# kwea123/nerf_pl

Hardware: AMD Instinct MI355X
Metric: rays/sec (64+128 samples), full training step: render_rays fwd + MSE + bwd + grad all-reduce + Adam (higher is better)
Workload: dtype bf16

## Files before the change

### nerf_pl_amd/csrc/composite_wave.h

```cpp
#pragma once
#include "loss_math.h"
#include "sampling_wave.h"

namespace nerfhip {

struct RayGeom {
    float dnorm;
};

__device__ __forceinline__ float ray_dnorm(const float* __restrict__ rays, int64_t r) {
    const float dx = rays[r * 8 + 3], dy = rays[r * 8 + 4], dz = rays[r * 8 + 5];
    return sqrtf(nh_add(nh_add(nh_mul(dx, dx), nh_mul(dy, dy)), nh_mul(dz, dz)));
}

struct SampleTerms {
    float delta;
    float e;
    float alpha;
    float sh;
    bool on;
};

__device__ __forceinline__ SampleTerms sample_terms(float z_i, float z_next, bool last, float dnorm, float sigma,
                                                    float noise) {
    SampleTerms t;
    const float d = last ? 1e10f : nh_sub(z_next, z_i);
    t.delta = nh_mul(d, dnorm);
    const float s = nh_add(sigma, noise);
    t.on = s > 0.0f;
    const float sr = t.on ? s : 0.0f;
    t.e = expf(-nh_mul(t.delta, sr));
    t.alpha = nh_sub(1.0f, t.e);
    t.sh = nh_add(nh_sub(1.0f, t.alpha), 1e-10f);
    return t;
}

template <int RAW_CH>
__device__ __forceinline__ void composite_fwd_wave(const float* __restrict__ raw, const float* __restrict__ z,
                                                   const float* __restrict__ rays, const float* __restrict__ noise, float noise_std,
                                                   int white_back, float* __restrict__ weights, float* __restrict__ rgb,
                                                   float* __restrict__ depth, float* __restrict__ opacity, int64_t r, int S,
                                                   float* w_s, int lane) {
    const float dnorm = ray_dnorm(rays, r);
    const float* zr = z + r * S;
    double carry = 1.0;
    float acc_r = 0.f, acc_g = 0.f, acc_b = 0.f, acc_d = 0.f, acc_o = 0.f;
    for (int i0 = 0; i0 < S; i0 += 64) {
        const int i = i0 + lane;
        const bool valid = i < S;
        float sigma = 0.f, cr = 0.f, cg = 0.f, cb = 0.f, zi = 0.f, zn = 0.f, nz = 0.f;
        if (valid) {
            zi = zr[i];
            zn = (i + 1 < S) ? zr[i + 1] : zi;
            if (RAW_CH == 4) {
                const float4 v = reinterpret_cast<const float4*>(raw)[r * S + i];
                cr = v.x; cg = v.y; cb = v.z; sigma = v.w;
            } else {
                sigma = raw[r * S + i];
            }
            if (noise) nz = nh_mul(noise[r * S + i], noise_std);
        }
        const SampleTerms t = sample_terms(zi, zn, i == S - 1, dnorm, sigma, nz);
        const double f = valid ? (double)t.sh : 1.0;
        const double incl = wave_incl_prod(f, lane);
        double excl = __shfl_up(incl, 1, 64);
        if (lane == 0) excl = 1.0;
        const float T = (float)(excl * carry);
        carry = carry * __shfl(incl, 63, 64);
        const float w = valid ? nh_mul(t.alpha, T) : 0.0f;
        if (valid) {
            if (weights) weights[r * S + i] = w;
            if (w_s) w_s[i] = w;
        }
        acc_o += w;
        if (RAW_CH == 4) {
            acc_r += w * cr; acc_g += w * cg; acc_b += w * cb;
            acc_d += w * zi;
        }
    }
    acc_o = wave_sum(acc_o);
    if (RAW_CH == 4) {
        acc_r = wave_sum(acc_r); acc_g = wave_sum(acc_g); acc_b = wave_sum(acc_b); acc_d = wave_sum(acc_d);
    }
    if (lane == 0) {
        if (opacity) opacity[r] = acc_o;
        if (RAW_CH == 4) {
            const float bg = white_back ? nh_sub(1.0f, acc_o) : 0.0f;
            if (rgb) {
                rgb[r * 3 + 0] = acc_r + bg;
                rgb[r * 3 + 1] = acc_g + bg;
                rgb[r * 3 + 2] = acc_b + bg;
            }
            if (depth) depth[r] = acc_d;
        }
    }
}

template <bool RGB_THROUGH = false>
__device__ __forceinline__ void composite_train_wave(const float* __restrict__ raw, const float* __restrict__ z,
                                                     const float* __restrict__ rays, const float* __restrict__ noise,
                                                     float noise_std, int white_back, const float* __restrict__ target,
                                                     float gscale, float* __restrict__ weights, float* __restrict__ rgb,
                                                     float* __restrict__ depth, float* __restrict__ opacity,
                                                     float* __restrict__ g_raw, int64_t r, int S, float* T_s, float* w_s, int lane) {
    const float dnorm = ray_dnorm(rays, r);
    const float* zr = z + r * S;
    double carry = 1.0;
    float acc_r = 0.f, acc_g = 0.f, acc_b = 0.f, acc_d = 0.f, acc_o = 0.f;
    for (int i0 = 0; i0 < S; i0 += 64) {
        const int i = i0 + lane;
        const bool valid = i < S;
        float sigma = 0.f, cr = 0.f, cg = 0.f, cb = 0.f, zi = 0.f, zn = 0.f, nz = 0.f;
        if (valid) {
            zi = zr[i];
            zn = (i + 1 < S) ? zr[i + 1] : zi;
            const float4 v = reinterpret_cast<const float4*>(raw)[r * S + i];
            cr = v.x; cg = v.y; cb = v.z; sigma = v.w;
            if (noise) nz = nh_mul(noise[r * S + i], noise_std);
        }
        const SampleTerms t = sample_terms(zi, zn, i == S - 1, dnorm, sigma, nz);
        const double f = valid ? (double)t.sh : 1.0;
        const double incl = wave_incl_prod(f, lane);
        double excl = __shfl_up(incl, 1, 64);
        if (lane == 0) excl = 1.0;
        const float T = (float)(excl * carry);
        carry = carry * __shfl(incl, 63, 64);
        const float w = valid ? nh_mul(t.alpha, T) : 0.0f;
        if (valid) {
            if (weights) weights[r * S + i] = w;
            if (w_s) w_s[i] = w;
            T_s[i] = T;
        }
        acc_o += w;
        acc_r += w * cr; acc_g += w * cg; acc_b += w * cb;
        acc_d += w * zi;
    }
    acc_o = wave_sum(acc_o);
    acc_r = wave_sum(acc_r); acc_g = wave_sum(acc_g); acc_b = wave_sum(acc_b); acc_d = wave_sum(acc_d);
    const float bg = white_back ? nh_sub(1.0f, acc_o) : 0.0f;
    const float out_r = acc_r + bg, out_g = acc_g + bg, out_b = acc_b + bg;
    if (lane == 0) {
        opacity[r] = acc_o;
        if (RGB_THROUGH) {
            __hip_atomic_store(rgb + r * 3 + 0, out_r, __ATOMIC_RELAXED, __HIP_MEMORY_SCOPE_AGENT);
            __hip_atomic_store(rgb + r * 3 + 1, out_g, __ATOMIC_RELAXED, __HIP_MEMORY_SCOPE_AGENT);
            __hip_atomic_store(rgb + r * 3 + 2, out_b, __ATOMIC_RELAXED, __HIP_MEMORY_SCOPE_AGENT);
        } else {
            rgb[r * 3 + 0] = out_r;
            rgb[r * 3 + 1] = out_g;
            rgb[r * 3 + 2] = out_b;
        }
        depth[r] = acc_d;
    }
    const float gr = nh_mul(nh_sub(out_r, target[r * 3]), gscale);
    const float gg = nh_mul(nh_sub(out_g, target[r * 3 + 1]), gscale);
    const float gb = nh_mul(nh_sub(out_b, target[r * 3 + 2]), gscale);
    const float gd = 0.f;
    float gconst = 0.f;
    if (white_back) gconst -= (gr + gg + gb);
    __builtin_amdgcn_wave_barrier();
    float tail = 0.f;
    const int nchunk = (S + 63) / 64;
    for (int c = nchunk - 1; c >= 0; --c) {
        const int i = c * 64 + lane;
        const bool valid = i < S;
        SampleTerms t{};
        float T = 0.f, gw = 0.f;
        if (valid) {
            const float zi = zr[i];
            const float zn = (i + 1 < S) ? zr[i + 1] : zi;
            const float4 v = reinterpret_cast<const float4*>(raw)[r * S + i];
            const float nz = noise ? nh_mul(noise[r * S + i], noise_std) : 0.f;
            t = sample_terms(zi, zn, i == S - 1, dnorm, v.w, nz);
            T = T_s[i];
            const float w = t.alpha * T;
            gw = gconst + 0.f;
            gw += gr * v.x + gg * v.y + gb * v.z + gd * zi;
            float* o = g_raw + (r * S + i) * 4;
            o[0] = w * gr; o[1] = w * gg; o[2] = w * gb;
        }
        const float vv = valid ? gw * (t.alpha * T) : 0.f;
        float incl = vv;
#pragma unroll
        for (int o = 1; o < 64; o <<= 1) {
            const float tt = __shfl_down(incl, o, 64);
            if (lane + o < 64) incl += tt;
        }
        const float suf = (incl - vv) + tail;
        tail += __shfl(incl, 0, 64);
        if (valid) {
            const float g_alpha = gw * T - suf / t.sh;
            const float g_sigma = t.on ? g_alpha * t.delta * t.e : 0.f;
            g_raw[(r * S + i) * 4 + 3] = g_sigma;
        }
    }
}

template <int RAW_CH = 4>
__device__ __forceinline__ void composite_weights_wave(const float* __restrict__ raw, const float* __restrict__ z,
                                                       const float* __restrict__ rays, const float* __restrict__ noise,
                                                       float noise_std, int64_t r, int S, float* w_s, int lane) {
    const float dnorm = ray_dnorm(rays, r);
    const float* zr = z + r * S;
    double carry = 1.0;
    for (int i0 = 0; i0 < S; i0 += 64) {
        const int i = i0 + lane;
        const bool valid = i < S;
        float sigma = 0.f, zi = 0.f, zn = 0.f, nz = 0.f;
        if (valid) {
            zi = zr[i];
            zn = (i + 1 < S) ? zr[i + 1] : zi;
            sigma = RAW_CH == 4 ? raw[(r * S + i) * 4 + 3] : raw[r * S + i];
            if (noise) nz = nh_mul(noise[r * S + i], noise_std);
        }
        const SampleTerms t = sample_terms(zi, zn, i == S - 1, dnorm, sigma, nz);
        const double f = valid ? (double)t.sh : 1.0;
        const double incl = wave_incl_prod(f, lane);
        double excl = __shfl_up(incl, 1, 64);
        if (lane == 0) excl = 1.0;
        const float T = (float)(excl * carry);
        carry = carry * __shfl(incl, 63, 64);
        if (valid) w_s[i] = nh_mul(t.alpha, T);
    }
}

}
```

### nerf_pl_amd/csrc/mlp_render_kernel.h

```cpp
#pragma once
#include "composite_wave.h"
#include "mlp_fwd_kernel.h"

namespace nerfhip {

constexpr int kRenderRays = 4;

typedef nerfhip_render_args RenderArgs;

__host__ __device__ inline int render_tail_floats(int S_c, int N_i, int S_f) {
    const int S4 = (S_c + 3) & ~3, N4 = (N_i + 3) & ~3, F4 = (S_f + 3) & ~3;
    const int fz = N_i > 0 ? 3 * S4 + N4 + ((S_c + 1 + 3) & ~3) + N4 : 0;
    const int coarse = 2 * S4 + fz;
    return coarse > F4 ? coarse : F4;
}

__device__ __forceinline__ void render_wg_sync() {
    asm volatile("s_waitcnt vmcnt(0) lgkmcnt(0)\n\ts_barrier" ::: "memory");
}

typedef const RenderArgs __attribute__((address_space(4)))* RenderArgsP;
__device__ __forceinline__ RenderArgsP render_args() {
    RenderArgsP p = (RenderArgsP)__builtin_amdgcn_kernarg_segment_ptr();
    asm volatile("" : "+s"(p));
    return p;
}

template <bool TRAIN, int NW, bool TT = false>
__device__ __forceinline__ void render_tail(const bool fine_pass, const bool with_fine_z, float* const tail_lds, const int wave,
                                            const int lane) {
    constexpr int R = kRenderRays;
    const RenderArgsP a = render_args();
    const int S_c = a->S_c, N_i = a->N_i, S_f = S_c + N_i;
    const float noise_std = a->noise_std;
    const float* raw = fine_pass ? a->raw_fine : a->raw_coarse;
    const float* z = fine_pass ? a->z_fine : a->z_coarse;
    const float* noise = noise_std != 0.0f ? (fine_pass ? a->noise_fine : a->noise_coarse) : nullptr;
    const int S = fine_pass ? S_f : S_c;
    float* rgb = fine_pass ? a->rgb_fine : a->rgb_coarse;
    float* depth = fine_pass ? a->depth_fine : a->depth_coarse;
    float* opac = fine_pass ? a->opacity_fine : a->opacity_coarse;
    const float* rays = a->rays;
    const int white_back = a->white_back;
    const int per_ray = render_tail_floats(S_c, N_i, S_f);
    const int S4 = (S_c + 3) & ~3;
    const int64_t ray0 = (int64_t)blockIdx.x * R, B = a->B;
    const int njobs = with_fine_z ? 2 * R : R;
    for (int job = wave; job < njobs; job += NW) {
        const int slot = job < R ? job : job - R;
        const int64_t r = ray0 + slot;
        if (r >= B) continue;
        float* base = tail_lds + (size_t)slot * per_ray;
        if (job < R) {
            if constexpr (TRAIN) {
                composite_train_wave<true>(raw, z, rays, noise, noise_std, white_back, a->target, a->grad_scale, nullptr, rgb, depth, opac,
                                           fine_pass ? a->g_raw_fine : a->g_raw_coarse, r, S, base, nullptr, lane);
            } else if (TT && !fine_pass) {
                composite_fwd_wave<1>(raw, z, rays, noise, noise_std, white_back, nullptr, nullptr, nullptr, opac, r, S, nullptr, lane);
            } else {
                composite_fwd_wave<4>(raw, z, rays, noise, noise_std, white_back, nullptr, rgb, depth, opac, r, S, nullptr, lane);
            }
        } else {
            float* w_s = base + S4;
            composite_weights_wave<(TT ? 1 : 4)>(raw, z, rays, noise, noise_std, r, S, w_s, lane);
            __builtin_amdgcn_wave_barrier();
            const float* u = a->u;
            fine_z_wave(w_s + S4, z + r * S, [&](int j) { return w_s[1 + j]; }, u ? u + r * a->u_stride : nullptr, S, N_i, a->eps,
                        a->z_fine + r * S_f, nullptr, nullptr, nullptr, lane, a->row_total);
        }
    }
}

template <int PREC, int SV>
__global__ __launch_bounds__(PrecTraits<PREC>::NW * 64, PrecTraits<PREC>::WPS)
void mlp_render_kernel(const RenderArgs args_by_value) {
    constexpr bool TRAIN = SV == 1 || SV == 2, TT = SV == 3;
    constexpr int FSV = TT ? 0 : SV;
    constexpr int NW = PrecTraits<PREC>::NW, PTS = 32 * NW, R = kRenderRays;
    __shared__ __attribute__((aligned(1024))) char lds_all[FwdLds<PREC, TRAIN>::kBytes];
    __shared__ float red[2][16];
    __shared__ unsigned last_s;
    const int lane = threadIdx.x & 63;
    const int wave = __builtin_amdgcn_readfirstlane((int)(threadIdx.x >> 6));
    float* const tail_lds = reinterpret_cast<float*>(lds_all + FwdLds<PREC, TRAIN>::kRingOff);
    int nc, nf;
    {
        const RenderArgsP a = render_args();
        const int S_c = a->S_c, N_i = a->N_i;
        nc = R * S_c / PTS;
        nf = N_i > 0 ? R * (S_c + N_i) / PTS : 0;
    }
    const int total = nc + nf;
#pragma clang loop unroll(disable)
    for (int sp = 0; sp < total; ++sp) {
        if (sp > 0) render_wg_sync();
        if (sp == nc) {
            render_tail<TRAIN, NW, TT>(false, true, tail_lds, wave, lane);
            render_wg_sync();
        }
        const RenderArgsP a = render_args();
        const bool fine = sp >= nc;
        const int S = fine ? a->S_c + a->N_i : a->S_c;
        const unsigned blk = fine ? blockIdx.x * (unsigned)nf + (unsigned)(sp - nc) : blockIdx.x * (unsigned)nc + (unsigned)sp;
        const FwdZGen zg{fine ? nullptr : a->perturb_rand, fine ? nullptr : a->z_coarse, fine ? 0 : a->use_disp, fine ? 0.0f : a->perturb,
                          TRAIN ? a->regen_enc : 0};
        uint8_t* save = nullptr;
        if constexpr (TRAIN) save = (uint8_t*)(fine ? a->save_fine : a->save_coarse);
        if (TT && !fine)
            mlp_fwd_body<PREC, MODE_RAYS, true, 0>(lds_all, blk, a->rays, nullptr, a->B * (int64_t)S, (int64_t)S, (const uint8_t*)a->packed_coarse,
                                                   a->raw_coarse, nullptr, zg);
        else
            mlp_fwd_body<PREC, MODE_RAYS, false, FSV>(lds_all, blk, a->rays, fine ? a->z_fine : nullptr, a->B * (int64_t)S, (int64_t)S,
                                                      (const uint8_t*)(fine ? a->packed_fine : a->packed_coarse), fine ? a->raw_fine : a->raw_coarse, save, zg);
    }
    render_wg_sync();
    render_tail<TRAIN, NW, TT>(nf > 0, false, tail_lds, wave, lane);

    if constexpr (TRAIN) {
        const RenderArgsP a = render_args();
        unsigned* const ticket = a->ticket;
        asm volatile("s_waitcnt vmcnt(0)" ::: "memory");
        __syncthreads();
        if (threadIdx.x == 0) {
            const unsigned prev = __hip_atomic_fetch_add(ticket, 1u, __ATOMIC_RELAXED, __HIP_MEMORY_SCOPE_AGENT);
            last_s = (prev == gridDim.x - 1) ? 1u : 0u;
            if (prev == gridDim.x - 1) __hip_atomic_store(ticket, 0u, __ATOMIC_RELAXED, __HIP_MEMORY_SCOPE_AGENT);
        }
        __syncthreads();
        if (!last_s) return;
        __builtin_amdgcn_fence(__ATOMIC_ACQUIRE, "agent");
        const float* img_c = a->rgb_coarse;
        const float* img_f = a->rgb_fine;
        const float* target = a->target;
        float* out3 = a->out3;
        const int64_t n3 = 3 * a->B;
        auto fresh_c = [&](int64_t i) { return __hip_atomic_load(img_c + i, __ATOMIC_RELAXED, __HIP_MEMORY_SCOPE_AGENT); };
        auto fresh_f = [&](int64_t i) { return __hip_atomic_load(img_f + i, __ATOMIC_RELAXED, __HIP_MEMORY_SCOPE_AGENT); };
        constexpr int Q = 1024 / (NW * 64);
        if (nf > 0)
            mse_psnr_block<Q>(fresh_c, fresh_f, true, target, n3, out3, nullptr, nullptr, red);
        else
            mse_psnr_block<Q>(fresh_c, [&](int64_t i) { return 0.0f; }, false, target, n3, out3, nullptr, nullptr, red);
    }
}

template <int PREC, int SV>
int launch_render_variant(const RenderArgs& a, unsigned groups, hipStream_t stream);

}
```

### nerf_pl_amd/csrc/optim.hip

```cpp
#include "adam_math.h"

namespace nerfhip {

constexpr int kAdamMaxTensors = 8;
struct AdamTable {
    float* param[kAdamMaxTensors];
    const float* grad[kAdamMaxTensors];
    float* m[kAdamMaxTensors];
    float* v[kAdamMaxTensors];
    int64_t n[kAdamMaxTensors];
    int block0[kAdamMaxTensors + 1];
    int count;
};

constexpr int kAdamThreads = 256, kAdamVec = 4, kAdamPerBlock = kAdamThreads * kAdamVec * 4;

__device__ __forceinline__ void advance_step(float* state, float t) {
    __syncthreads();
    if (threadIdx.x == 0) {
        unsigned* ticket = reinterpret_cast<unsigned*>(state + 1);
        const unsigned prev = atomicAdd(ticket, 1u);
        if (prev == gridDim.x - 1) {
            *ticket = 0u;
            state[0] = t;
        }
    }
}

__global__ __launch_bounds__(kAdamThreads) void adam_kernel(AdamTable T, float* __restrict__ state, float lr, float beta1,
                                                            float beta2, float eps, float wd) {
    const float t = state[0] + 1.0f;
    int ti = 0;
#pragma unroll
    for (int k = 1; k < kAdamMaxTensors; ++k) ti += (k < T.count && (int)blockIdx.x >= T.block0[k]) ? 1 : 0;
    const int64_t base = (int64_t)((int)blockIdx.x - T.block0[ti]) * kAdamPerBlock;
    const int64_t n = T.n[ti];
    float* __restrict__ P = T.param[ti];
    const float* __restrict__ G = T.grad[ti];
    float* __restrict__ M = T.m[ti];
    float* __restrict__ V = T.v[ti];
    const AdamCoef ac = adam_coef(t, lr, beta1, beta2);
#pragma unroll
    for (int r = 0; r < 4; ++r) {
        const int64_t i = base + ((int64_t)r * kAdamThreads + threadIdx.x) * kAdamVec;
        if (i + kAdamVec <= n && ((((uintptr_t)(P + i)) | ((uintptr_t)(G + i)) | ((uintptr_t)(M + i)) | ((uintptr_t)(V + i))) & 15) == 0) {
            float4 p = *reinterpret_cast<const float4*>(P + i), g = *reinterpret_cast<const float4*>(G + i);
            float4 m = *reinterpret_cast<const float4*>(M + i), v = *reinterpret_cast<const float4*>(V + i);
            float* pp = &p.x; float* gp = &g.x; float* mp = &m.x; float* vp = &v.x;
#pragma unroll
            for (int k = 0; k < 4; ++k) adam_elem(pp[k], gp[k], mp[k], vp[k], ac, beta2, eps, wd);
            *reinterpret_cast<float4*>(P + i) = p;
            *reinterpret_cast<float4*>(M + i) = m;
            *reinterpret_cast<float4*>(V + i) = v;
        } else {
            for (int k = 0; k < kAdamVec; ++k) {
                const int64_t j = i + k;
                if (j < n) adam_elem(P[j], G[j], M[j], V[j], ac, beta2, eps, wd);
            }
        }
    }
    __syncthreads();
    if (threadIdx.x == 0) {
        unsigned* ticket = reinterpret_cast<unsigned*>(state + 1);
        const unsigned prev = atomicAdd(ticket, 1u);
        if (prev == gridDim.x - 1) {
            *ticket = 0u;
            state[0] = t;
        }
    }
}

struct SlowTable {
    float* slow[kAdamMaxTensors];
};

struct RadamCoef {
    float step_lr;
    float wd_lr;
    float beta1, beta2, omb1, omb2, eps, alpha;
    int mode;
    bool decay, sync, init;
};

template <bool kRanger>
__device__ __forceinline__ RadamCoef radam_coef(float t, double lr, double beta1, double beta2, double eps, double wd, double alpha,
                                                int k, double threshold, int degenerated_to_sgd) {
    RadamCoef c;
    const double td = (double)t;
    const double beta2_t = pow(beta2, td);
    const double n_max = 2.0 / (1.0 - beta2) - 1.0;
    const double n_sma = n_max - 2.0 * td * beta2_t / (1.0 - beta2_t);
    const double bc1 = 1.0 - pow(beta1, td);
    const bool rectified = kRanger ? (n_sma > threshold) : (n_sma >= threshold);
    double step_size;
    if (rectified) {
        step_size = sqrt((1.0 - beta2_t) * (n_sma - 4.0) / (n_max - 4.0) * (n_sma - 2.0) / n_sma * n_max / (n_max - 2.0)) / bc1;
        c.mode = 2;
    } else {
        step_size = 1.0 / bc1;
        c.mode = (kRanger || degenerated_to_sgd) ? 1 : 0;
    }
    c.step_lr = (float)(-step_size * lr);
    c.wd_lr = (float)(-wd * lr);
    c.decay = wd != 0.0;
    c.beta1 = (float)beta1;
    c.beta2 = (float)beta2;
    c.omb1 = (float)(1.0 - beta1);
    c.omb2 = (float)(1.0 - beta2);
    c.eps = (float)eps;
    c.alpha = (float)alpha;
    c.sync = kRanger && ((int)t % k == 0);
    c.init = kRanger && t == 1.0f;
    return c;
}

template <bool kRanger>
__device__ __forceinline__ void radam_elem(float& p, float g, float& m, float& v, float& s, const RadamCoef& c) {
    v = v * c.beta2 + c.omb2 * g * g;
    m = m * c.beta1 + c.omb1 * g;
    if (c.mode == 0) return;
    float q = p;
    if (kRanger && c.init) s = q;
    if (c.decay) q = q + c.wd_lr * q;
    q = (c.mode == 2) ? q + c.step_lr * (m / (sqrtf(v) + c.eps)) : q + c.step_lr * m;
    if (kRanger && c.sync) {
        s = s + c.alpha * (q - s);
        q = s;
    }
    p = q;
}

template <bool kRanger>
__global__ __launch_bounds__(kAdamThreads) void radam_kernel(AdamTable T, SlowTable ST, float* __restrict__ state, double lr,
                                                             double beta1, double beta2, double eps, double wd, double alpha, int k,
                                                             double threshold, int degenerated_to_sgd) {
    const float t = state[0] + 1.0f;
    int ti = 0;
#pragma unroll
    for (int j = 1; j < kAdamMaxTensors; ++j) ti += (j < T.count && (int)blockIdx.x >= T.block0[j]) ? 1 : 0;
    const int64_t base = (int64_t)((int)blockIdx.x - T.block0[ti]) * kAdamPerBlock;
    const int64_t n = T.n[ti];
    float* __restrict__ P = T.param[ti];
    const float* __restrict__ G = T.grad[ti];
    float* __restrict__ M = T.m[ti];
    float* __restrict__ V = T.v[ti];
    const RadamCoef c = radam_coef<kRanger>(t, lr, beta1, beta2, eps, wd, alpha, k, threshold, degenerated_to_sgd);
    const bool slow_rd = kRanger && c.sync && !c.init, slow_wr = kRanger && (c.sync || c.init);
    float* __restrict__ S = slow_wr ? ST.slow[ti] : nullptr;
#pragma unroll
    for (int r = 0; r < 4; ++r) {
        const int64_t i = base + ((int64_t)r * kAdamThreads + threadIdx.x) * kAdamVec;
        uintptr_t align = ((uintptr_t)(P + i)) | ((uintptr_t)(G + i)) | ((uintptr_t)(M + i)) | ((uintptr_t)(V + i));
        if (slow_wr) align |= (uintptr_t)(S + i);
        if (i + kAdamVec <= n && (align & 15) == 0) {
            float4 p = *reinterpret_cast<const float4*>(P + i), g = *reinterpret_cast<const float4*>(G + i);
            float4 m = *reinterpret_cast<const float4*>(M + i), v = *reinterpret_cast<const float4*>(V + i);
            float4 s = make_float4(0.f, 0.f, 0.f, 0.f);
            if (slow_rd) s = *reinterpret_cast<const float4*>(S + i);
            float* pp = &p.x; float* gp = &g.x; float* mp = &m.x; float* vp = &v.x; float* sp = &s.x;
#pragma unroll
            for (int e = 0; e < 4; ++e) radam_elem<kRanger>(pp[e], gp[e], mp[e], vp[e], sp[e], c);
            if (c.mode != 0) *reinterpret_cast<float4*>(P + i) = p;
            *reinterpret_cast<float4*>(M + i) = m;
            *reinterpret_cast<float4*>(V + i) = v;
            if (slow_wr) *reinterpret_cast<float4*>(S + i) = s;
        } else {
            for (int e = 0; e < kAdamVec; ++e) {
                const int64_t j = i + e;
                if (j < n) {
                    float p = P[j], m = M[j], v = V[j], s = slow_rd ? S[j] : 0.f;
                    radam_elem<kRanger>(p, G[j], m, v, s, c);
                    if (c.mode != 0) P[j] = p;
                    M[j] = m;
                    V[j] = v;
                    if (slow_wr) S[j] = s;
                }
            }
        }
    }
    advance_step(state, t);
}

}

namespace nerfhip {

static int adam_table(AdamTable& T, int& blocks, float* const* params_host, const float* const* grads_host, float* const* exp_avg_host,
                      float* const* exp_avg_sq_host, const int64_t* numel_host, int n_tensors) {
    NERFHIP_CHECK_ARG(params_host && grads_host && exp_avg_host && exp_avg_sq_host && numel_host);
    NERFHIP_CHECK_ARG(n_tensors >= 1 && n_tensors <= kAdamMaxTensors);
    blocks = 0;
    for (int i = 0; i < n_tensors; ++i) {
        NERFHIP_CHECK_ARG(params_host[i] && grads_host[i] && exp_avg_host[i] && exp_avg_sq_host[i] && numel_host[i] > 0);
        T.param[i] = params_host[i];
        T.grad[i] = grads_host[i];
        T.m[i] = exp_avg_host[i];
        T.v[i] = exp_avg_sq_host[i];
        T.n[i] = numel_host[i];
        T.block0[i] = blocks;
        const int64_t nb = (numel_host[i] + kAdamPerBlock - 1) / kAdamPerBlock;
        if (nb + blocks > 0x3fffffff) return NERFHIP_E_BADARG;
        blocks += (int)nb;
    }
    for (int i = n_tensors; i < kAdamMaxTensors; ++i) {
        T.param[i] = nullptr; T.grad[i] = nullptr; T.m[i] = nullptr; T.v[i] = nullptr; T.n[i] = 0;
        T.block0[i] = blocks;
    }
    T.block0[kAdamMaxTensors] = blocks;
    T.count = n_tensors;
    return 0;
}

static bool radam_hyper_ok(double lr, double beta1, double beta2, double eps, double weight_decay) {
    return lr >= 0.0 && beta1 >= 0.0 && beta1 < 1.0 && beta2 >= 0.0 && beta2 < 1.0 && eps >= 0.0 && weight_decay >= 0.0;
}

}

extern "C" int nerfhip_adam_step(float* const* params_host, const float* const* grads_host, float* const* exp_avg_host,
                                 float* const* exp_avg_sq_host, const int64_t* numel_host, int n_tensors, float* state,
                                 float lr, float beta1, float beta2, float eps, float weight_decay, nerfhip_stream_t stream) {
    NERFHIP_CHECK_ARG(state);
    nerfhip::AdamTable T;
    int blocks = 0;
    const int rc = nerfhip::adam_table(T, blocks, params_host, grads_host, exp_avg_host, exp_avg_sq_host, numel_host, n_tensors);
    if (rc != 0) return rc;
    hipLaunchKernelGGL(nerfhip::adam_kernel, dim3(blocks), dim3(nerfhip::kAdamThreads), 0, (hipStream_t)stream, T, state, lr,
                       beta1, beta2, eps, weight_decay);
    return nerfhip_launch_status();
}

extern "C" int nerfhip_radam_step(float* const* params_host, const float* const* grads_host, float* const* exp_avg_host,
                                  float* const* exp_avg_sq_host, const int64_t* numel_host, int n_tensors, float* state,
                                  double lr, double beta1, double beta2, double eps, double weight_decay, int degenerated_to_sgd,
                                  nerfhip_stream_t stream) {
    NERFHIP_CHECK_ARG(state && nerfhip::radam_hyper_ok(lr, beta1, beta2, eps, weight_decay));
    nerfhip::AdamTable T;
    int blocks = 0;
    const int rc = nerfhip::adam_table(T, blocks, params_host, grads_host, exp_avg_host, exp_avg_sq_host, numel_host, n_tensors);
    if (rc != 0) return rc;
    nerfhip::SlowTable ST;
    for (int i = 0; i < nerfhip::kAdamMaxTensors; ++i) ST.slow[i] = nullptr;
    hipLaunchKernelGGL(nerfhip::radam_kernel<false>, dim3(blocks), dim3(nerfhip::kAdamThreads), 0, (hipStream_t)stream, T, ST, state,
                       lr, beta1, beta2, eps, weight_decay, 0.0, 1, 5.0, degenerated_to_sgd ? 1 : 0);
    return nerfhip_launch_status();
}

extern "C" int nerfhip_ranger_step(float* const* params_host, const float* const* grads_host, float* const* exp_avg_host,
                                   float* const* exp_avg_sq_host, const int64_t* numel_host, int n_tensors, float* state,
                                   float* const* slow_host, double alpha, int k, double n_sma_threshold, double lr, double beta1,
                                   double beta2, double eps, double weight_decay, nerfhip_stream_t stream) {
    NERFHIP_CHECK_ARG(state && slow_host && nerfhip::radam_hyper_ok(lr, beta1, beta2, eps, weight_decay));
    NERFHIP_CHECK_ARG(k >= 1 && alpha >= 0.0 && alpha <= 1.0);
    nerfhip::AdamTable T;
    int blocks = 0;
    const int rc = nerfhip::adam_table(T, blocks, params_host, grads_host, exp_avg_host, exp_avg_sq_host, numel_host, n_tensors);
    if (rc != 0) return rc;
    nerfhip::SlowTable ST;
    for (int i = 0; i < nerfhip::kAdamMaxTensors; ++i) {
        ST.slow[i] = i < n_tensors ? slow_host[i] : nullptr;
        NERFHIP_CHECK_ARG(i >= n_tensors || slow_host[i]);
    }
    hipLaunchKernelGGL(nerfhip::radam_kernel<true>, dim3(blocks), dim3(nerfhip::kAdamThreads), 0, (hipStream_t)stream, T, ST, state,
                       lr, beta1, beta2, eps, weight_decay, alpha, k, n_sma_threshold, 1);
    return nerfhip_launch_status();
}
```

Baseline: 1.096 million.

## Batch composite loads across sample chunks and hoist Adam loads ahead of math

The composite forward, train and weights routines now load several 64-sample chunks of z, raw and noise into registers up front (clamped indices, masked afterwards), instead of issuing guarded loads one chunk at a time. When all samples fit in one group, the backward pass reuses the registers filled by the forward pass rather than reloading from global memory. The Adam kernel gets a whole-block fast path that issues all 16 float4 loads before any math and pins them with empty asm to keep loads early, aiming to expose more memory-level parallelism. An optional timestamp probe is also added behind a compile flag that is off by default. The cost is higher register pressure, which may lower occupancy.

```diff
diff --git a/nerf_pl_amd/csrc/composite_wave.h b/nerf_pl_amd/csrc/composite_wave.h
--- a/nerf_pl_amd/csrc/composite_wave.h
+++ b/nerf_pl_amd/csrc/composite_wave.h
@@ -35,8 +35,42 @@
     return t;
 }
 
-template <int RAW_CH>
-__device__ __forceinline__ void composite_fwd_wave(const float* __restrict__ raw, const float* __restrict__ z,
+constexpr int kCompositeGroup = 4;
+template <int RAW_CH, int NC>
+struct CompositeChunks {
+    float4 v[NC];
+    float zi[NC], zn[NC], nz[NC];
+    template <bool SIGMA_ONLY, bool NOISE>
+    __device__ __forceinline__ void load_all(const float* __restrict__ raw, const float* __restrict__ zr, const float* __restrict__ noise,
+                                             float noise_std, int64_t r, int S, int g0, int lane) {
+#pragma unroll
+        for (int c = 0; c < NC; ++c) {
+            const int i = g0 + 64 * c + lane;
+            const int ic = i < S ? i : S - 1, in = i + 1 < S ? i + 1 : S - 1;
+            zi[c] = zr[ic];
+            zn[c] = zr[in];
+            if (RAW_CH == 4 && !SIGMA_ONLY) v[c] = reinterpret_cast<const float4*>(raw)[r * S + ic];
+            else v[c] = make_float4(0.f, 0.f, 0.f, RAW_CH == 4 ? raw[(r * S + ic) * 4 + 3] : raw[r * S + ic]);
+            nz[c] = NOISE ? noise[r * S + ic] : 0.f;
+        }
+#pragma unroll
+        for (int c = 0; c < NC; ++c) {
+            const bool valid = g0 + 64 * c + lane < S;
+            if (NOISE) nz[c] = nh_mul(nz[c], noise_std);
+            zi[c] = valid ? zi[c] : 0.f; zn[c] = valid ? zn[c] : 0.f; nz[c] = valid ? nz[c] : 0.f;
+            v[c].x = valid ? v[c].x : 0.f; v[c].y = valid ? v[c].y : 0.f; v[c].z = valid ? v[c].z : 0.f; v[c].w = valid ? v[c].w : 0.f;
+        }
+    }
+    template <bool SIGMA_ONLY = false>
+    __device__ __forceinline__ void load(const float* __restrict__ raw, const float* __restrict__ zr, const float* __restrict__ noise,
+                                         float noise_std, int64_t r, int S, int g0, int lane) {
+        if (noise) load_all<SIGMA_ONLY, true>(raw, zr, noise, noise_std, r, S, g0, lane);
+        else load_all<SIGMA_ONLY, false>(raw, zr, noise, noise_std, r, S, g0, lane);
+    }
+};
+
+template <int RAW_CH, int NC>
+__device__ __forceinline__ void composite_fwd_wave_impl(const float* __restrict__ raw, const float* __restrict__ z,
                                                    const float* __restrict__ rays, const float* __restrict__ noise, float noise_std,
                                                    int white_back, float* __restrict__ weights, float* __restrict__ rgb,
                                                    float* __restrict__ depth, float* __restrict__ opacity, int64_t r, int S,
@@ -45,37 +79,33 @@
     const float* zr = z + r * S;
     double carry = 1.0;
     float acc_r = 0.f, acc_g = 0.f, acc_b = 0.f, acc_d = 0.f, acc_o = 0.f;
-    for (int i0 = 0; i0 < S; i0 += 64) {
-        const int i = i0 + lane;
-        const bool valid = i < S;
-        float sigma = 0.f, cr = 0.f, cg = 0.f, cb = 0.f, zi = 0.f, zn = 0.f, nz = 0.f;
-        if (valid) {
-            zi = zr[i];
-            zn = (i + 1 < S) ? zr[i + 1] : zi;
+    CompositeChunks<RAW_CH, NC> in;
+    for (int g0 = 0; g0 < S; g0 += 64 * NC) {
+        in.load(raw, zr, noise, noise_std, r, S, g0, lane);
+#pragma unroll
+        for (int c = 0; c < NC; ++c) {
+            const int i0 = g0 + 64 * c;
+            if (i0 >= S) break;
+            const int i = i0 + lane;
+            const bool valid = i < S;
+            const float cr = in.v[c].x, cg = in.v[c].y, cb = in.v[c].z, sigma = in.v[c].w, zi = in.zi[c];
+            const SampleTerms t = sample_terms(zi, in.zn[c], i == S - 1, dnorm, sigma, in.nz[c]);
+            const double f = valid ? (double)t.sh : 1.0;
+            const double incl = wave_incl_prod(f, lane);
+            double excl = __shfl_up(incl, 1, 64);
+            if (lane == 0) excl = 1.0;
+            const float T = (float)(excl * carry);
+            carry = carry * __shfl(incl, 63, 64);
+            const float w = valid ? nh_mul(t.alpha, T) : 0.0f;
+            if (valid) {
+                if (weights) weights[r * S + i] = w;
+                if (w_s) w_s[i] = w;
+            }
+            acc_o += w;
             if (RAW_CH == 4) {
-                const float4 v = reinterpret_cast<const float4*>(raw)[r * S + i];
-                cr = v.x; cg = v.y; cb = v.z; sigma = v.w;
-            } else {
-                sigma = raw[r * S + i];
-            }
-            if (noise) nz = nh_mul(noise[r * S + i], noise_std);
-        }
-        const SampleTerms t = sample_terms(zi, zn, i == S - 1, dnorm, sigma, nz);
-        const double f = valid ? (double)t.sh : 1.0;
-        const double incl = wave_incl_prod(f, lane);
-        double excl = __shfl_up(incl, 1, 64);
-        if (lane == 0) excl = 1.0;
-        const float T = (float)(excl * carry);
-        carry = carry * __shfl(incl, 63, 64);
-        const float w = valid ? nh_mul(t.alpha, T) : 0.0f;
-        if (valid) {
-            if (weights) weights[r * S + i] = w;
-            if (w_s) w_s[i] = w;
-        }
-        acc_o += w;
-        if (RAW_CH == 4) {
-            acc_r += w * cr; acc_g += w * cg; acc_b += w * cb;
-            acc_d += w * zi;
+                acc_r += w * cr; acc_g += w * cg; acc_b += w * cb;
+                acc_d += w * zi;
+            }
         }
     }
     acc_o = wave_sum(acc_o);
@@ -95,9 +125,18 @@
         }
     }
 }
-
-template <bool RGB_THROUGH = false>
-__device__ __forceinline__ void composite_train_wave(const float* __restrict__ raw, const float* __restrict__ z,
+template <int RAW_CH>
+__device__ __forceinline__ void composite_fwd_wave(const float* __restrict__ raw, const float* __restrict__ z,
+                                                   const float* __restrict__ rays, const float* __restrict__ noise, float noise_std,
+                                                   int white_back, float* __restrict__ weights, float* __restrict__ rgb,
+                                                   float* __restrict__ depth, float* __restrict__ opacity, int64_t r, int S,
+                                                   float* w_s, int lane) {
+    if (S <= 64) composite_fwd_wave_impl<RAW_CH, 1>(raw, z, rays, noise, noise_std, white_back, weights, rgb, depth, opacity, r, S, w_s, lane);
+    else composite_fwd_wave_impl<RAW_CH, kCompositeGroup>(raw, z, rays, noise, noise_std, white_back, weights, rgb, depth, opacity, r, S, w_s, lane);
+}
+
+template <bool RGB_THROUGH, int NC>
+__device__ __forceinline__ void composite_train_wave_impl(const float* __restrict__ raw, const float* __restrict__ z,
                                                      const float* __restrict__ rays, const float* __restrict__ noise,
                                                      float noise_std, int white_back, const float* __restrict__ target,
                                                      float gscale, float* __restrict__ weights, float* __restrict__ rgb,
@@ -105,35 +144,37 @@
                                                      float* __restrict__ g_raw, int64_t r, int S, float* T_s, float* w_s, int lane) {
     const float dnorm = ray_dnorm(rays, r);
     const float* zr = z + r * S;
+    const float tgt_r = target[r * 3], tgt_g = target[r * 3 + 1], tgt_b = target[r * 3 + 2];
     double carry = 1.0;
     float acc_r = 0.f, acc_g = 0.f, acc_b = 0.f, acc_d = 0.f, acc_o = 0.f;
-    for (int i0 = 0; i0 < S; i0 += 64) {
-        const int i = i0 + lane;
-        const bool valid = i < S;
-        float sigma = 0.f, cr = 0.f, cg = 0.f, cb = 0.f, zi = 0.f, zn = 0.f, nz = 0.f;
-        if (valid) {
-            zi = zr[i];
-            zn = (i + 1 < S) ? zr[i + 1] : zi;
-            const float4 v = reinterpret_cast<const float4*>(raw)[r * S + i];
-            cr = v.x; cg = v.y; cb = v.z; sigma = v.w;
-            if (noise) nz = nh_mul(noise[r * S + i], noise_std);
-        }
-        const SampleTerms t = sample_terms(zi, zn, i == S - 1, dnorm, sigma, nz);
-        const double f = valid ? (double)t.sh : 1.0;
-        const double incl = wave_incl_prod(f, lane);
-        double excl = __shfl_up(incl, 1, 64);
-        if (lane == 0) excl = 1.0;
-        const float T = (float)(excl * carry);
-        carry = carry * __shfl(incl, 63, 64);
-        const float w = valid ? nh_mul(t.alpha, T) : 0.0f;
-        if (valid) {
-            if (weights) weights[r * S + i] = w;
-            if (w_s) w_s[i] = w;
-            T_s[i] = T;
-        }
-        acc_o += w;
-        acc_r += w * cr; acc_g += w * cg; acc_b += w * cb;
-        acc_d += w * zi;
+    CompositeChunks<4, NC> in;
+    const bool one_group = S <= 64 * NC;
+    for (int g0 = 0; g0 < S; g0 += 64 * NC) {
+        in.load(raw, zr, noise, noise_std, r, S, g0, lane);
+#pragma unroll
+        for (int c = 0; c < NC; ++c) {
+            const int i0 = g0 + 64 * c;
+            if (i0 >= S) break;
+            const int i = i0 + lane;
+            const bool valid = i < S;
+            const float cr = in.v[c].x, cg = in.v[c].y, cb = in.v[c].z, sigma = in.v[c].w, zi = in.zi[c];
+            const SampleTerms t = sample_terms(zi, in.zn[c], i == S - 1, dnorm, sigma, in.nz[c]);
+            const double f = valid ? (double)t.sh : 1.0;
+            const double incl = wave_incl_prod(f, lane);
+            double excl = __shfl_up(incl, 1, 64);
+            if (lane == 0) excl = 1.0;
+            const float T = (float)(excl * carry);
+            carry = carry * __shfl(incl, 63, 64);
+            const float w = valid ? nh_mul(t.alpha, T) : 0.0f;
+            if (valid) {
+                if (weights) weights[r * S + i] = w;
+                if (w_s) w_s[i] = w;
+                T_s[i] = T;
+            }
+            acc_o += w;
+            acc_r += w * cr; acc_g += w * cg; acc_b += w * cb;
+            acc_d += w * zi;
+        }
     }
     acc_o = wave_sum(acc_o);
     acc_r = wave_sum(acc_r); acc_g = wave_sum(acc_g); acc_b = wave_sum(acc_b); acc_d = wave_sum(acc_d);
@@ -152,76 +193,102 @@
         }
         depth[r] = acc_d;
     }
-    const float gr = nh_mul(nh_sub(out_r, target[r * 3]), gscale);
-    const float gg = nh_mul(nh_sub(out_g, target[r * 3 + 1]), gscale);
-    const float gb = nh_mul(nh_sub(out_b, target[r * 3 + 2]), gscale);
+    const float gr = nh_mul(nh_sub(out_r, tgt_r), gscale);
+    const float gg = nh_mul(nh_sub(out_g, tgt_g), gscale);
+    const float gb = nh_mul(nh_sub(out_b, tgt_b), gscale);
     const float gd = 0.f;
     float gconst = 0.f;
     if (white_back) gconst -= (gr + gg + gb);
     __builtin_amdgcn_wave_barrier();
     float tail = 0.f;
-    const int nchunk = (S + 63) / 64;
-    for (int c = nchunk - 1; c >= 0; --c) {
-        const int i = c * 64 + lane;
-        const bool valid = i < S;
-        SampleTerms t{};
-        float T = 0.f, gw = 0.f;
-        if (valid) {
-            const float zi = zr[i];
-            const float zn = (i + 1 < S) ? zr[i + 1] : zi;
-            const float4 v = reinterpret_cast<const float4*>(raw)[r * S + i];
-            const float nz = noise ? nh_mul(noise[r * S + i], noise_std) : 0.f;
-            t = sample_terms(zi, zn, i == S - 1, dnorm, v.w, nz);
-            T = T_s[i];
-            const float w = t.alpha * T;
-            gw = gconst + 0.f;
-            gw += gr * v.x + gg * v.y + gb * v.z + gd * zi;
-            float* o = g_raw + (r * S + i) * 4;
-            o[0] = w * gr; o[1] = w * gg; o[2] = w * gb;
-        }
-        const float vv = valid ? gw * (t.alpha * T) : 0.f;
-        float incl = vv;
-#pragma unroll
-        for (int o = 1; o < 64; o <<= 1) {
-            const float tt = __shfl_down(incl, o, 64);
-            if (lane + o < 64) incl += tt;
-        }
-        const float suf = (incl - vv) + tail;
-        tail += __shfl(incl, 0, 64);
-        if (valid) {
-            const float g_alpha = gw * T - suf / t.sh;
-            const float g_sigma = t.on ? g_alpha * t.delta * t.e : 0.f;
-            g_raw[(r * S + i) * 4 + 3] = g_sigma;
-        }
-    }
-}
-
-template <int RAW_CH = 4>
-__device__ __forceinline__ void composite_weights_wave(const float* __restrict__ raw, const float* __restrict__ z,
+    const int ngroup = (S + 64 * NC - 1) / (64 * NC);
+    for (int g = ngroup - 1; g >= 0; --g) {
+        const int g0 = g * 64 * NC;
+        if (!one_group) in.load(raw, zr, noise, noise_std, r, S, g0, lane);
+#pragma unroll
+        for (int c = NC - 1; c >= 0; --c) {
+            const int i0 = g0 + 64 * c;
+            if (i0 >= S) continue;
+            const int i = i0 + lane;
+            const bool valid = i < S;
+            SampleTerms t{};
+            float T = 0.f, gw = 0.f;
+            if (valid) {
+                const float zi = in.zi[c];
+                const float4 v = in.v[c];
+                t = sample_terms(zi, in.zn[c], i == S - 1, dnorm, v.w, in.nz[c]);
+                T = T_s[i];
+                const float w = t.alpha * T;
+                gw = gconst + 0.f;
+                gw += gr * v.x + gg * v.y + gb * v.z + gd * zi;
+                float* o = g_raw + (r * S + i) * 4;
+                o[0] = w * gr; o[1] = w * gg; o[2] = w * gb;
+            }
+            const float vv = valid ? gw * (t.alpha * T) : 0.f;
+            float incl = vv;
+#pragma unroll
+            for (int o = 1; o < 64; o <<= 1) {
+                const float tt = __shfl_down(incl, o, 64);
+                if (lane + o < 64) incl += tt;
+            }
+            const float suf = (incl - vv) + tail;
+            tail += __shfl(incl, 0, 64);
+            if (valid) {
+                const float g_alpha = gw * T - suf / t.sh;
+                const float g_sigma = t.on ? g_alpha * t.delta * t.e : 0.f;
+                g_raw[(r * S + i) * 4 + 3] = g_sigma;
+            }
+        }
+    }
+}
+template <bool RGB_THROUGH = false>
+__device__ __forceinline__ void composite_train_wave(const float* __restrict__ raw, const float* __restrict__ z,
+                                                     const float* __restrict__ rays, const float* __restrict__ noise,
+                                                     float noise_std, int white_back, const float* __restrict__ target,
+                                                     float gscale, float* __restrict__ weights, float* __restrict__ rgb,
+                                                     float* __restrict__ depth, float* __restrict__ opacity,
+                                                     float* __restrict__ g_raw, int64_t r, int S, float* T_s, float* w_s, int lane) {
+    if (S <= 64)
+        composite_train_wave_impl<RGB_THROUGH, 1>(raw, z, rays, noise, noise_std, white_back, target, gscale, weights, rgb, depth, opacity, g_raw,
+                                                  r, S, T_s, w_s, lane);
+    else
+        composite_train_wave_impl<RGB_THROUGH, kCompositeGroup>(raw, z, rays, noise, noise_std, white_back, target, gscale, weights, rgb, depth,
+                                                                opacity, g_raw, r, S, T_s, w_s, lane);
+}
+
+template <int RAW_CH, int NC>
+__device__ __forceinline__ void composite_weights_wave_impl(const float* __restrict__ raw, const float* __restrict__ z,
                                                        const float* __restrict__ rays, const float* __restrict__ noise,
                                                        float noise_std, int64_t r, int S, float* w_s, int lane) {
     const float dnorm = ray_dnorm(rays, r);
     const float* zr = z + r * S;
     double carry = 1.0;
-    for (int i0 = 0; i0 < S; i0 += 64) {
-        const int i = i0 + lane;
-        const bool valid = i < S;
-        float sigma = 0.f, zi = 0.f, zn = 0.f, nz = 0.f;
-        if (valid) {
-            zi = zr[i];
-            zn = (i + 1 < S) ? zr[i + 1] : zi;
-            sigma = RAW_CH == 4 ? raw[(r * S + i) * 4 + 3] : raw[r * S + i];
-            if (noise) nz = nh_mul(noise[r * S + i], noise_std);
-        }
-        const SampleTerms t = sample_terms(zi, zn, i == S - 1, dnorm, sigma, nz);
-        const double f = valid ? (double)t.sh : 1.0;
-        const double incl = wave_incl_prod(f, lane);
-        double excl = __shfl_up(incl, 1, 64);
-        if (lane == 0) excl = 1.0;
-        const float T = (float)(excl * carry);
-        carry = carry * __shfl(incl, 63, 64);
-        if (valid) w_s[i] = nh_mul(t.alpha, T);
-    }
-}
-
-}
+    CompositeChunks<RAW_CH, NC> in;
+    for (int g0 = 0; g0 < S; g0 += 64 * NC) {
+        in.template load<true>(raw, zr, noise, noise_std, r, S, g0, lane);
+#pragma unroll
+        for (int c = 0; c < NC; ++c) {
+            const int i0 = g0 + 64 * c;
+            if (i0 >= S) break;
+            const int i = i0 + lane;
+            const bool valid = i < S;
+            const SampleTerms t = sample_terms(in.zi[c], in.zn[c], i == S - 1, dnorm, in.v[c].w, in.nz[c]);
+            const double f = valid ? (double)t.sh : 1.0;
+            const double incl = wave_incl_prod(f, lane);
+            double excl = __shfl_up(incl, 1, 64);
+            if (lane == 0) excl = 1.0;
+            const float T = (float)(excl * carry);
+            carry = carry * __shfl(incl, 63, 64);
+            if (valid) w_s[i] = nh_mul(t.alpha, T);
+        }
+    }
+}
+template <int RAW_CH = 4>
+__device__ __forceinline__ void composite_weights_wave(const float* __restrict__ raw, const float* __restrict__ z,
+                                                       const float* __restrict__ rays, const float* __restrict__ noise,
+                                                       float noise_std, int64_t r, int S, float* w_s, int lane) {
+    if (S <= 64) composite_weights_wave_impl<RAW_CH, 1>(raw, z, rays, noise, noise_std, r, S, w_s, lane);
+    else composite_weights_wave_impl<RAW_CH, kCompositeGroup>(raw, z, rays, noise, noise_std, r, S, w_s, lane);
+}
+
+}
diff --git a/nerf_pl_amd/csrc/mlp_render_kernel.h b/nerf_pl_amd/csrc/mlp_render_kernel.h
--- a/nerf_pl_amd/csrc/mlp_render_kernel.h
+++ b/nerf_pl_amd/csrc/mlp_render_kernel.h
@@ -5,6 +5,16 @@
 namespace nerfhip {
 
 constexpr int kRenderRays = 4;
+
+#ifndef NERFHIP_SEAM_PROBE
+#define NERFHIP_SEAM_PROBE 0
+#endif
+#if NERFHIP_SEAM_PROBE
+constexpr int kSeamStamps = 24;
+#define NERFHIP_SEAM_STAMP(k) do { if (lane == 0) seam_s[wave][(k)] = (unsigned)__builtin_amdgcn_s_memrealtime(); } while (0)
+#else
+#define NERFHIP_SEAM_STAMP(k) do { } while (0)
+#endif
 
 typedef nerfhip_render_args RenderArgs;
 
@@ -82,6 +92,11 @@
     __shared__ unsigned last_s;
     const int lane = threadIdx.x & 63;
     const int wave = __builtin_amdgcn_readfirstlane((int)(threadIdx.x >> 6));
+#if NERFHIP_SEAM_PROBE
+    __shared__ unsigned seam_s[NW][kSeamStamps];
+    if (lane < kSeamStamps) seam_s[wave][lane] = 0u;
+    NERFHIP_SEAM_STAMP(0);
+#endif
     float* const tail_lds = reinterpret_cast<float*>(lds_all + FwdLds<PREC, TRAIN>::kRingOff);
     int nc, nf;
     {
@@ -95,8 +110,11 @@
     for (int sp = 0; sp < total; ++sp) {
         if (sp > 0) render_wg_sync();
         if (sp == nc) {
+            NERFHIP_SEAM_STAMP(9);
             render_tail<TRAIN, NW, TT>(false, true, tail_lds, wave, lane);
+            NERFHIP_SEAM_STAMP(10);
             render_wg_sync();
+            NERFHIP_SEAM_STAMP(11);
         }
         const RenderArgsP a = render_args();
         const bool fine = sp >= nc;
@@ -106,27 +124,42 @@
                           TRAIN ? a->regen_enc : 0};
         uint8_t* save = nullptr;
         if constexpr (TRAIN) save = (uint8_t*)(fine ? a->save_fine : a->save_coarse);
+        if (sp < 4) NERFHIP_SEAM_STAMP(1 + 2 * sp);
         if (TT && !fine)
             mlp_fwd_body<PREC, MODE_RAYS, true, 0>(lds_all, blk, a->rays, nullptr, a->B * (int64_t)S, (int64_t)S, (const uint8_t*)a->packed_coarse,
                                                    a->raw_coarse, nullptr, zg);
         else
             mlp_fwd_body<PREC, MODE_RAYS, false, FSV>(lds_all, blk, a->rays, fine ? a->z_fine : nullptr, a->B * (int64_t)S, (int64_t)S,
                                                       (const uint8_t*)(fine ? a->packed_fine : a->packed_coarse), fine ? a->raw_fine : a->raw_coarse, save, zg);
+        if (sp < 4) NERFHIP_SEAM_STAMP(2 + 2 * sp);
     }
     render_wg_sync();
+    NERFHIP_SEAM_STAMP(12);
     render_tail<TRAIN, NW, TT>(nf > 0, false, tail_lds, wave, lane);
+    NERFHIP_SEAM_STAMP(13);
 
     if constexpr (TRAIN) {
         const RenderArgsP a = render_args();
         unsigned* const ticket = a->ticket;
         asm volatile("s_waitcnt vmcnt(0)" ::: "memory");
+        NERFHIP_SEAM_STAMP(14);
         __syncthreads();
+        NERFHIP_SEAM_STAMP(15);
         if (threadIdx.x == 0) {
             const unsigned prev = __hip_atomic_fetch_add(ticket, 1u, __ATOMIC_RELAXED, __HIP_MEMORY_SCOPE_AGENT);
             last_s = (prev == gridDim.x - 1) ? 1u : 0u;
             if (prev == gridDim.x - 1) __hip_atomic_store(ticket, 0u, __ATOMIC_RELAXED, __HIP_MEMORY_SCOPE_AGENT);
         }
         __syncthreads();
+        NERFHIP_SEAM_STAMP(16);
+#if NERFHIP_SEAM_PROBE
+        auto seam_flush = [&]() {
+            __builtin_amdgcn_wave_barrier();
+            if (lane < kSeamStamps)
+                reinterpret_cast<unsigned*>(a->g_raw_coarse)[(size_t)blockIdx.x * (R * 64 * 4) + wave * 32 + lane] = seam_s[wave][lane];
+        };
+        if (!last_s) seam_flush();
+#endif
         if (!last_s) return;
         __builtin_amdgcn_fence(__ATOMIC_ACQUIRE, "agent");
         const float* img_c = a->rgb_coarse;
@@ -141,6 +174,10 @@
             mse_psnr_block<Q>(fresh_c, fresh_f, true, target, n3, out3, nullptr, nullptr, red);
         else
             mse_psnr_block<Q>(fresh_c, [&](int64_t i) { return 0.0f; }, false, target, n3, out3, nullptr, nullptr, red);
+#if NERFHIP_SEAM_PROBE
+        NERFHIP_SEAM_STAMP(17);
+        seam_flush();
+#endif
     }
 }
 
diff --git a/nerf_pl_amd/csrc/optim.hip b/nerf_pl_amd/csrc/optim.hip
--- a/nerf_pl_amd/csrc/optim.hip
+++ b/nerf_pl_amd/csrc/optim.hip
@@ -27,6 +27,8 @@
     }
 }
 
+__device__ __forceinline__ void pin_loaded(float4& a) { asm volatile("" : "+v"(a.x), "+v"(a.y), "+v"(a.z), "+v"(a.w)); }
+
 __global__ __launch_bounds__(kAdamThreads) void adam_kernel(AdamTable T, float* __restrict__ state, float lr, float beta1,
                                                             float beta2, float eps, float wd) {
     const float t = state[0] + 1.0f;
@@ -39,23 +41,48 @@
     const float* __restrict__ G = T.grad[ti];
     float* __restrict__ M = T.m[ti];
     float* __restrict__ V = T.v[ti];
-    const AdamCoef ac = adam_coef(t, lr, beta1, beta2);
-#pragma unroll
-    for (int r = 0; r < 4; ++r) {
-        const int64_t i = base + ((int64_t)r * kAdamThreads + threadIdx.x) * kAdamVec;
-        if (i + kAdamVec <= n && ((((uintptr_t)(P + i)) | ((uintptr_t)(G + i)) | ((uintptr_t)(M + i)) | ((uintptr_t)(V + i))) & 15) == 0) {
-            float4 p = *reinterpret_cast<const float4*>(P + i), g = *reinterpret_cast<const float4*>(G + i);
-            float4 m = *reinterpret_cast<const float4*>(M + i), v = *reinterpret_cast<const float4*>(V + i);
-            float* pp = &p.x; float* gp = &g.x; float* mp = &m.x; float* vp = &v.x;
+    const int64_t i0 = base + (int64_t)threadIdx.x * kAdamVec;
+    constexpr int64_t kRow = (int64_t)kAdamThreads * kAdamVec;
+    const bool whole = base + kAdamPerBlock <= n &&
+                       ((((uintptr_t)(P + base)) | ((uintptr_t)(G + base)) | ((uintptr_t)(M + base)) | ((uintptr_t)(V + base))) & 15) == 0;
+    if (whole) {
+        float4 p[4], g[4], m[4], v[4];
+#pragma unroll
+        for (int r = 0; r < 4; ++r) {
+            p[r] = *reinterpret_cast<const float4*>(P + i0 + r * kRow); g[r] = *reinterpret_cast<const float4*>(G + i0 + r * kRow);
+            m[r] = *reinterpret_cast<const float4*>(M + i0 + r * kRow); v[r] = *reinterpret_cast<const float4*>(V + i0 + r * kRow);
+        }
+#pragma unroll
+        for (int r = 0; r < 4; ++r) { pin_loaded(p[r]); pin_loaded(g[r]); pin_loaded(m[r]); pin_loaded(v[r]); }
+        const AdamCoef ac = adam_coef(t, lr, beta1, beta2);
+#pragma unroll
+        for (int r = 0; r < 4; ++r) {
+            float* pp = &p[r].x; float* gp = &g[r].x; float* mp = &m[r].x; float* vp = &v[r].x;
 #pragma unroll
             for (int k = 0; k < 4; ++k) adam_elem(pp[k], gp[k], mp[k], vp[k], ac, beta2, eps, wd);
-            *reinterpret_cast<float4*>(P + i) = p;
-            *reinterpret_cast<float4*>(M + i) = m;
-            *reinterpret_cast<float4*>(V + i) = v;
-        } else {
-            for (int k = 0; k < kAdamVec; ++k) {
-                const int64_t j = i + k;
-                if (j < n) adam_elem(P[j], G[j], M[j], V[j], ac, beta2, eps, wd);
+            *reinterpret_cast<float4*>(P + i0 + r * kRow) = p[r];
+            *reinterpret_cast<float4*>(M + i0 + r * kRow) = m[r];
+            *reinterpret_cast<float4*>(V + i0 + r * kRow) = v[r];
+        }
+    } else {
+        const AdamCoef ac = adam_coef(t, lr, beta1, beta2);
+#pragma unroll
+        for (int r = 0; r < 4; ++r) {
+            const int64_t i = i0 + r * kRow;
+            if (i + kAdamVec <= n && ((((uintptr_t)(P + i)) | ((uintptr_t)(G + i)) | ((uintptr_t)(M + i)) | ((uintptr_t)(V + i))) & 15) == 0) {
+                float4 p = *reinterpret_cast<const float4*>(P + i), g = *reinterpret_cast<const float4*>(G + i);
+                float4 m = *reinterpret_cast<const float4*>(M + i), v = *reinterpret_cast<const float4*>(V + i);
+                float* pp = &p.x; float* gp = &g.x; float* mp = &m.x; float* vp = &v.x;
+#pragma unroll
+                for (int k = 0; k < 4; ++k) adam_elem(pp[k], gp[k], mp[k], vp[k], ac, beta2, eps, wd);
+                *reinterpret_cast<float4*>(P + i) = p;
+                *reinterpret_cast<float4*>(M + i) = m;
+                *reinterpret_cast<float4*>(V + i) = v;
+            } else {
+                for (int k = 0; k < kAdamVec; ++k) {
+                    const int64_t j = i + k;
+                    if (j < n) adam_elem(P[j], G[j], M[j], V[j], ac, beta2, eps, wd);
+                }
             }
         }
     }
```

New measurement: 1.107 million (median of 3 runs). Within noise of the previous version (+1.0%).
